# EPFL-IMOS/simple-SFOD

Measured on AMD Instinct MI355X. Metric: teacher+student train images/s on 1024x2048 synthetic, higher is better.
Workload: dtype bf16x3

## Files before the change

include/sfod_hip.h:

```cpp
#ifndef SFOD_HIP_H
#define SFOD_HIP_H
#include <stdint.h>
#ifdef __cplusplus
extern "C" {
#endif

#define SFOD_F32 0
#define SFOD_BF16 1
#define SFOD_BF16X3 2
#define SFOD_F16X3 3

int sfod_version(void);
const char* sfod_last_error(void);

int sfod_preprocess(const void* const* img_ptrs, const int32_t* sizes, int B, int Hp, int Wp,
                    int Cpad, const float* mean3, const float* std3, void* out, int dt,
                    void* stream);

int sfod_hflip_u8(const void* src, void* dst, int C, int H, int W, void* stream);

int sfod_resize_bilinear_u8(const void* src, void* dst, int C, int H, int W, int h, int w,
                            const int32_t* hbounds, const int32_t* hcoef, int ksize_h,
                            const int32_t* vbounds, const int32_t* vcoef, int ksize_v, int flip,
                            void* stream);
// ... 11 lines not shown
int sfod_conv_fwd_ws(const void* x, const void* w, const uint32_t* w_absmax, const float* bias, void* y, int B, int H,
                     int W, int Cin, int Cout, int ksize, int ldy, int act, float* stats, int dt, int out_dt,
                     void* stream);
int64_t sfod_conv_fwd_scratch_bytes(int B, int H, int W, int Cin, int Cout, int ksize, int dt, int out_dt, int with_stats);
int sfod_conv_fwd_scratch(const void* x, const void* w, const uint32_t* w_absmax, const float* bias, void* y, int B, int H,
                          int W, int Cin, int Cout, int ksize, int ldy, int act, float* stats, int dt, int out_dt,
                          void* scratch, int64_t scratch_bytes, void* stream);
int sfod_conv_stats_blocks(int B, int H, int W, int Cin, int Cout, int ksize, int dt);
int sfod_set_conv_algo(int algo);
int sfod_conv_dgrad_bnred_blocks(int B, int H, int W, int Cin, int Cout, int dt);
int sfod_conv_dgrad_bnred(const void* x, const void* w, void* dz, int B, int H, int W, int Cin, int Cout, int dt,
                          const float* y, const float* mean, const float* invstd, const float* gamma,
                          const float* beta, float* red_ws, void* stream);
int sfod_conv_fwd_bnin_supported(int B, int H, int W, int Cin, int Cout, int dt);
int sfod_conv_fwd_bnin(const float* x_pre, const float* in_mean, const float* in_invstd, const float* in_gamma,
                       const float* in_beta, const void* w, const float* bias, float* y, int B, int H, int W, int Cin,
                       int Cout, int ldy, int act, float* stats, int dt, void* stream);
int sfod_set_gemm_tile(int tile);
int sfod_set_conv3x3_variant(int variant);
int sfod_last_conv_kernel(char* buf, int n);
int sfod_set_deterministic(int on);
int sfod_get_deterministic(void);
int sfod_set_conv3x3_m16(int on);
int sfod_set_wgrad3x3_pipe(int on);
int sfod_conv_fwd_algo(int B, int H, int W, int Cin, int Cout, int ksize, int dt);

int sfod_conv_first_supported(int B, int H, int W, int Cin, int Cout, int dt, int ldy);
int sfod_conv_first_fused(const void* x, const void* w, const float* bias, const float* scale,
                          const float* shift, void* y, float* stats, int B, int H, int W, int ldy,
                          int act, int dt, void* stream);
int sfod_conv_first_fused_ws(const void* x, const void* w, const uint32_t* w_absmax, const float* bias,
                             const float* scale, const float* shift, void* y, float* stats, int B, int H, int W,
                             int ldy, int act, int dt, void* stream);

int64_t sfod_conv_wgrad_ws_bytes(int B, int H, int W, int Cin, int Cout, int ksize, int lddy, int dt);
int sfod_conv_wgrad(const void* x, const void* dy, float* dw, int B, int H, int W, int Cin,
                    int Cout, int ksize, int lddy, int dt, void* ws, int64_t ws_bytes, void* stream);
int sfod_conv_wgrad_oihw_supported(int B, int H, int W, int Cin, int Cout, int ksize, int lddy, int dt);
int sfod_conv_wgrad_oihw(const void* x, const void* dy, float* dw_oihw, int B, int H, int W, int Cin,
                         int Cout, int ksize, int lddy, int dt, int accumulate, void* ws,
                         int64_t ws_bytes, void* stream);
int sfod_conv_first_wgrad_bn_supported(int B, int H, int W, int Cin, int Cout, int pool, int dt, int y_dt);
int sfod_conv_first_wgrad_bn(const void* x, const void* dz, const void* y, const float* mean, const float* invstd,
                             const float* gamma, const float* beta, const float* dgamma, const float* dbeta,
                             float* dw, int B, int H, int W, int Cin, int Cout, int dt, int oihw, int accumulate,
                             void* ws, int64_t ws_bytes, void* stream);
int sfod_set_first_wgrad_fused(int on);

int sfod_pack_conv_weight(const float* w_oihw, void* w_packed, int Cout, int Cin, int ksize,
                          int CinPad, int rot180, int dt, void* stream);
int sfod_pack_conv_weight_ws(const float* w_oihw, void* w_packed, uint32_t* absmax, int Cout, int Cin, int ksize,
                             int CinPad, int rot180, int dt, void* stream);
int sfod_pack_conv_weights_blocks(int Cout, int Cin, int ksize, int innerPad, int rot180);
int sfod_pack_conv_weights_multi(const int64_t* desc, int n, int total_blocks, int dt, void* stream);
int sfod_pack_conv_weights_multi_ws(const int64_t* desc, int n, int total_blocks, int dt, uint32_t* absmax ,
                                    void* stream);
int sfod_unpack_conv_wgrad(const float* dw_packed, float* dw_oihw, int Cout, int Cin, int ksize,
                           int CinPad, int accumulate, void* stream);
int sfod_pack_fc_weight(const float* w, void* out, int N, int K, int chw_c, int transpose, int dt,
                        void* stream);
int sfod_unpack_fc_wgrad(const float* dw_packed, float* dw, int N, int K, int chw_c,
                         int accumulate, void* stream);
int sfod_pack_fc_weight_ld(const float* w, void* out, int N, int K, int chw_c, int transpose, int ld,
                           int dt, void* stream);
int sfod_pack_fc_weight_ld_ws(const float* w, void* out, uint32_t* absmax, int N, int K, int chw_c, int transpose,
                              int ld, int dt, void* stream);
// ... 251 lines not shown
```

simple-sfod_amd/csrc/conv_first.hip:

```cpp
#include "conv_internal.h"
#include <type_traits>

typedef __attribute__((ext_vector_type(8))) __bf16 bf16x8;
typedef __attribute__((ext_vector_type(16))) float f32x16;

namespace {

constexpr int TH = 8, TW = 32, PW = TW + 2, PH = TH + 2;
constexpr int PATCH_BYTES = PH * PW * 16;
constexpr int STG_OFF = 5632;
constexpr int STG_PITCH = 144;
constexpr int SRED_OFF = STG_OFF + 4 * 64 * STG_PITCH;
constexpr int LDS_BYTES = SRED_OFF + 4 * 64 * 2 * 4 + 16;
constexpr int X3_PATCH_BYTES = PH * PW * 32;
constexpr int X3_W_OFF = 11008;
constexpr int X3_W_BYTES = 5 * 2 * 2 * 64 * 16;
constexpr int X3_STG_OFF = X3_W_OFF + X3_W_BYTES;
constexpr int X3_FP = 272;
constexpr int X3_SRED_OFF = X3_STG_OFF + 4 * 16 * X3_FP;
constexpr int X3_LDS_BYTES = X3_SRED_OFF + 4 * 64 * 2 * 4 + 16;

struct F1Args {
  const bf16_t* x;
  const bf16_t* w;
  const float* bias;
  const float* scale;
  const float* shift;
  void* y;
  float* stats;
  int B, H, W, ldy, act;
  int tiles_y, tiles_x, ntiles;
  const unsigned* wamax;
};

__global__ void __launch_bounds__(256)
k_conv_first(F1Args a) {
  __shared__ __attribute__((aligned(16))) unsigned char smem[LDS_BYTES];
  const int lane = threadIdx.x & 63;
  const int wave = __builtin_amdgcn_readfirstlane(threadIdx.x >> 6);
  const int h = lane >> 5, l31 = lane & 31;

  bf16x8 bq[2][5];
#pragma unroll
  for (int j = 0; j < 2; ++j)
#pragma unroll
    for (int s = 0; s < 5; ++s) {
      const int tap = 2 * s + h;
      uint4 v = make_uint4(0, 0, 0, 0);
      if (tap < 9) v = *reinterpret_cast<const uint4*>(a.w + ((j * 32 + l31) * 9 + tap) * 8);
      bq[j][s] = __builtin_bit_cast(bf16x8, v);
    }
  float bcol[2], scol[2], hcol[2];
#pragma unroll
  for (int j = 0; j < 2; ++j) {
    bcol[j] = a.bias ? a.bias[j * 32 + l31] : 0.f;
    scol[j] = a.scale ? a.scale[j * 32 + l31] : 1.f;
    hcol[j] = a.shift ? a.shift[j * 32 + l31] : 0.f;
  }
  const float lo = (a.act == 1) ? 0.f : -__builtin_inff();

  for (int tile = blockIdx.x; tile < a.ntiles; tile += gridDim.x) {
    int t = tile;
    const int txi = t % a.tiles_x;
    t /= a.tiles_x;
    const int tyi = t % a.tiles_y;
// ... 115 lines not shown
        }
        q += __shfl_xor(q, 32);
        if (h == 0) {
          sred[(wave * 64 + j * 32 + l31) * 2 + 0] = sm;
          sred[(wave * 64 + j * 32 + l31) * 2 + 1] = q;
        }
      }
      if (lane == 0) scnt[wave] = (float)cnt;
      __syncthreads();
      if (threadIdx.x < 64) {
        const int col = threadIdx.x;
        double n_tot = 0.0, s_tot = 0.0;
#pragma unroll
        for (int k = 0; k < 4; ++k) { n_tot += (double)scnt[k]; s_tot += (double)sred[(k * 64 + col) * 2]; }
        const double mu = n_tot > 0.0 ? s_tot / n_tot : 0.0;
        double m2 = 0.0;
#pragma unroll
        for (int k = 0; k < 4; ++k) {
          const double nk = (double)scnt[k];
          if (nk > 0.0) {
            const double d = (double)sred[(k * 64 + col) * 2] / nk - mu;
            m2 += (double)sred[(k * 64 + col) * 2 + 1] + nk * d * d;
          }
        }
        a.stats[((int64_t)tile * 2 + 0) * 64 + col] = (float)s_tot;
        a.stats[((int64_t)tile * 2 + 1) * 64 + col] = (float)m2;
        if (col == 0) a.stats[(int64_t)a.ntiles * 2 * 64 + tile] = (float)n_tot;
      }
    }
  }
}

template <int FMT>
__global__ void __launch_bounds__(256) __attribute__((amdgpu_waves_per_eu(3, 3)))
k_conv_first_x3(F1Args a) {
  using pair_t = typename std::conditional<FMT == 2, splith_t, split_t>::type;
  const float winv = (FMT == 2 && a.wamax != nullptr) ? winv_from_absmax(*a.wamax) : 1.0f;
  __shared__ __attribute__((aligned(16))) unsigned char smem[X3_LDS_BYTES];
  const int lane = threadIdx.x & 63;
  const int wave = __builtin_amdgcn_readfirstlane(threadIdx.x >> 6);
  const int h = lane >> 5, l31 = lane & 31;
  for (int e = threadIdx.x; e < 5 * 2 * 64; e += 256) {
    const int ln = e & 63, j = (e >> 6) & 1, ks = e >> 7;
    const int tap = 2 * ks + (ln >> 5);
    uint4 vh = make_uint4(0, 0, 0, 0), vl = vh;
    if (tap < 9) {
      const uint4* p = reinterpret_cast<const uint4*>(a.w + ((j * 32 + (ln & 31)) * 9 + tap) * 16);
      vh = p[0];
      vl = p[1];
    }
    *reinterpret_cast<uint4*>(smem + X3_W_OFF + (((ks * 2 + j) * 2 + 0) * 64 + ln) * 16) = vh;
    *reinterpret_cast<uint4*>(smem + X3_W_OFF + (((ks * 2 + j) * 2 + 1) * 64 + ln) * 16) = vl;
  }
  float bcol[2], scol[2], hcol[2];
#pragma unroll
  for (int j = 0; j < 2; ++j) {
    bcol[j] = a.bias ? a.bias[j * 32 + l31] : 0.f;
    scol[j] = a.scale ? a.scale[j * 32 + l31] : 1.f;
    hcol[j] = a.shift ? a.shift[j * 32 + l31] : 0.f;
  }
  const float lo = (a.act == 1) ? 0.f : -__builtin_inff();
  const bool zsplit = (a.scale != nullptr);

  for (int tile = blockIdx.x; tile < a.ntiles; tile += gridDim.x) {
    int t = tile;
    const int txi = t % a.tiles_x;
    t /= a.tiles_x;
    const int tyi = t % a.tiles_y;
    const int b = t / a.tiles_y;
    const int x0 = txi * TW, y0 = tyi * TH;
    const bf16_t* ximg = a.x + (int64_t)b * a.H * a.W * 16;
// ... 128 lines not shown
            q += ((vmask[i] >> r) & 1u) ? d * d : 0.f;
          }
        q += __shfl_xor(q, 32);
        if (h == 0) {
          sred[(wave * 64 + j * 32 + l31) * 2 + 0] = sm;
          sred[(wave * 64 + j * 32 + l31) * 2 + 1] = q;
        }
      }
      if (lane == 0) scnt[wave] = (float)cnt;
      __syncthreads();
      if (threadIdx.x < 64) {
        const int col = threadIdx.x;
        double n_tot = 0.0, s_tot = 0.0;
#pragma unroll
        for (int k = 0; k < 4; ++k) { n_tot += (double)scnt[k]; s_tot += (double)sred[(k * 64 + col) * 2]; }
        const double mu = n_tot > 0.0 ? s_tot / n_tot : 0.0;
        double m2 = 0.0;
#pragma unroll
        for (int k = 0; k < 4; ++k) {
          const double nk = (double)scnt[k];
          if (nk > 0.0) {
            const double d = (double)sred[(k * 64 + col) * 2] / nk - mu;
            m2 += (double)sred[(k * 64 + col) * 2 + 1] + nk * d * d;
          }
        }
        a.stats[((int64_t)tile * 2 + 0) * 64 + col] = (float)s_tot;
        a.stats[((int64_t)tile * 2 + 1) * 64 + col] = (float)m2;
        if (col == 0) a.stats[(int64_t)a.ntiles * 2 * 64 + tile] = (float)n_tot;
      }
    }
  }
}

}

int sfod_f1_nblk(int B, int H, int W) { return B * ((H + TH - 1) / TH) * ((W + TW - 1) / TW); }

int sfod_f1_launch(const void* x, const void* w, const float* bias, void* y, float* stats, int B, int H, int W,
                   int ldy, int act, hipStream_t s, const float* scale, const float* shift, int split, const unsigned* wamax) {
  F1Args a;
  a.wamax = wamax;
  a.x = (const bf16_t*)x; a.w = (const bf16_t*)w; a.bias = bias; a.y = y; a.stats = stats;
  a.scale = scale; a.shift = shift;
  a.B = B; a.H = H; a.W = W; a.ldy = ldy; a.act = act;
  a.tiles_y = (H + TH - 1) / TH; a.tiles_x = (W + TW - 1) / TW;
  a.ntiles = B * a.tiles_y * a.tiles_x;
  const int resident = split ? 256 * 3 : 256 * 8;
  int grid = a.ntiles < resident ? a.ntiles : resident;
  sfod_note_conv_kernel(split == 2 ? "k_conv_first_x3<2>" : (split ? "k_conv_first_x3<1>" : "k_conv_first"));
  if (split == 2) hipLaunchKernelGGL(k_conv_first_x3<2>, dim3(grid), dim3(256), 0, s, a);
  else if (split) hipLaunchKernelGGL(k_conv_first_x3<1>, dim3(grid), dim3(256), 0, s, a);
  else hipLaunchKernelGGL(k_conv_first, dim3(grid), dim3(256), 0, s, a);
  return sfod_check_launch("conv_first");
}

SFOD_DEFINE_F16_POLL(sfod_f16_poll_first)
```

simple-sfod_amd/csrc/conv_internal.h:

```cpp
#pragma once
#include "common.h"

struct P3Plan {
  int ok;
  int G;
  int FM;
  int TH, TW;
  int tiles_y, tiles_x, tiles_n;
  int nblk;
  int m16;
};
P3Plan sfod_p3_plan(int B, int H, int W, int Cin, int Cout, int pairs = 0);
struct P3BnRed {
  const float* y;
  const float* mean;
  const float* invstd;
  const float* gamma;
  const float* beta;
  float* ws;
};
struct P3BnIn {
  const float* mean;
  const float* invstd;
  const float* gamma;
// ... 12 lines not shown
  int co_tiles, ci_tiles;
  int tiles_per_split, nsplit, nslab;
  int64_t ws_bytes;
  int w64;
};
W3Plan sfod_w3_plan(int B, int H, int W, int Cin, int Cout, int lddy, int split = 0);
int sfod_w3_launch(const W3Plan& p, const void* x, const void* dy, float* dw, void* ws, int B, int H, int W,
                   int Cin, int Cout, int lddy, int out_mode, hipStream_t s, int split = 0);

struct W3BnApply {
  const float* dz;
  const float* y;
  const float* mean;
  const float* invstd;
  const float* gamma;
  const float* beta;
  const float* dgamma;
  const float* dbeta;
};
bool sfod_w3_bn_ok(const W3Plan& p, int Cin, int Cout);
int sfod_w3_bn_launch(const W3Plan& p, const void* x, const W3BnApply& bn, float* dw, void* ws, int B, int H, int W,
                      int out_mode, hipStream_t s);

bool sfod_deterministic();

void sfod_f16_poll_elementwise(unsigned* out, hipStream_t s);
void sfod_f16_poll_roi(unsigned* out, hipStream_t s);
void sfod_f16_poll_first(unsigned* out, hipStream_t s);
void sfod_f16_poll_stem(unsigned* out, hipStream_t s);
void sfod_f16_poll_gn(unsigned* out, hipStream_t s);
void sfod_f16_poll_cda(unsigned* out, hipStream_t s);

int sfod_f1_nblk(int B, int H, int W);
int sfod_f1_launch(const void* x, const void* w, const float* bias, void* y, float* stats, int B, int H, int W,
                   int ldy, int act, hipStream_t s, const float* scale = nullptr, const float* shift = nullptr, int split = 0,
                   const unsigned* wamax = nullptr);
```

simple-sfod_amd/csrc/gemm_conv.hip:

```cpp
#include "conv_internal.h"
#include <algorithm>

typedef __attribute__((ext_vector_type(8))) __bf16 bf16x8;
typedef __attribute__((ext_vector_type(4))) short s16x4;
typedef __attribute__((ext_vector_type(8))) short s16x8;
typedef __attribute__((ext_vector_type(16))) float f32x16;
typedef __attribute__((ext_vector_type(4))) float f32x4;

#define LDS_PTR(p) ((__attribute__((address_space(3))) void*)(p))
#define GLB_PTR(p) ((const __attribute__((address_space(1))) void*)(p))

__device__ __attribute__((aligned(16))) unsigned int g_zero_page[64];

struct ConvArgs {
  int M;
  int H, W;
  int Cin;
  int Cout;
  int ks;
  int cpt_shift;
  int kchunks;
  int ldy;
  int act;
  const unsigned* wamax;
// ... 625 lines not shown
    }
  }
#undef TILE
  sfod_set_error("conv_fwd: tile shape %d is not built for these operands", (int)tile);
  return SFOD_EBADARG;
}

template <typename T, typename OutT, int SPLIT = 0>
static int launch_conv_fwd(const ConvFwdPlan& p, const void* x, const void* w, const float* bias, void* y, float* stats,
                           const ConvArgs& a, hipStream_t s) {
  if (p.ut) return launch_tile<T, OutT, true, SPLIT>(p.tile, x, w, bias, y, stats, a, s);
  return launch_tile<T, OutT, false, SPLIT>(p.tile, x, w, bias, y, stats, a, s);
}

extern "C" int sfod_conv_first_supported(int B, int H, int W, int Cin, int Cout, int dt, int ldy) {
  if (!(conv_shape_fits(B, H, W, Cin, Cout, 3) && sfod_ints_ok({ldy}))) return 0;
  return conv_fwd_plan(B, H, W, Cin, Cout, 3, dt, sfod_is_pairs(dt) ? SFOD_F32 : dt, ldy, true, 0).kind == CONV_FIRST ? 1 : 0;
}

extern "C" int sfod_conv_first_fused(const void* x, const void* w, const float* bias, const float* scale,
                                     const float* shift, void* y, float* stats, int B, int H, int W, int ldy,
                                     int act, int dt, void* stream) {
  SFOD_REQUIRE_EXTENTS("conv_first_fused", B, H, W, ldy);
  return sfod_conv_first_fused_ws(x, w, nullptr, bias, scale, shift, y, stats, B, H, W, ldy, act, dt, stream);
}

extern "C" int sfod_conv_first_fused_ws(const void* x, const void* w, const uint32_t* w_absmax, const float* bias,
                                        const float* scale, const float* shift, void* y, float* stats, int B, int H,
                                        int W, int ldy, int act, int dt, void* stream) {
  sfod_note_conv_kernel(nullptr);
  SFOD_REQUIRE(conv_shape_fits(B, H, W, 8, 64, 3) && sfod_ints_ok({ldy}), "conv_first_fused: negative or oversized extent");
  SFOD_REQUIRE(x != nullptr && w != nullptr, "conv_first_fused: null operand");
  SFOD_REQUIRE(w_absmax == nullptr || dt == SFOD_F16X3, "conv_first: scaled weights are an SFOD_F16X3 format");
  SFOD_REQUIRE(sfod_conv_first_supported(B, H, W, 8, 64, dt, ldy),
               "conv_first_fused: shape not served by the first-layer kernel (sfod_conv_first_supported)");
  SFOD_REQUIRE(y != nullptr || stats != nullptr, "conv_first_fused: nothing to produce");
  SFOD_REQUIRE((scale == nullptr) == (shift == nullptr), "conv_first_fused: scale and shift come together");
  return sfod_f1_launch(x, w, bias, y, stats, B, H, W, ldy, act, (hipStream_t)stream, scale, shift, split_code(dt), w_absmax);
}

extern "C" int sfod_conv_fwd_scratch(const void* x, const void* w, const uint32_t* w_absmax, const float* bias, void* y,
                                     int B, int H, int W, int Cin, int Cout, int ksize, int ldy, int act, float* stats,
                                     int dt, int out_dt, void* scratch, int64_t scratch_bytes, void* stream) {
  sfod_note_conv_kernel(nullptr);
  SFOD_REQUIRE(conv_shape_fits(B, H, W, Cin, Cout, ksize) && sfod_ints_ok({ldy}) && sfod_i64s_ok({scratch_bytes}),
               "conv_fwd: negative or oversized extent");
  SFOD_REQUIRE(x != nullptr && w != nullptr && y != nullptr, "conv_fwd: null operand (x, w, y)");
  SFOD_REQUIRE(act >= 0 && act <= 2, "conv_fwd: unknown act");
  SFOD_REQUIRE(out_dt == SFOD_F32 || out_dt == SFOD_BF16 || sfod_is_pairs(out_dt), "conv_fwd: unknown out_dt");
  SFOD_REQUIRE(w_absmax == nullptr || dt == SFOD_F16X3, "conv: scaled weights are an SFOD_F16X3 format");
  SFOD_REQUIRE(ksize == 1 || ksize == 3, "conv: ksize must be 1 or 3");
  SFOD_REQUIRE(ldy >= Cout, "conv: ldy < Cout");
  const int E = (dt == SFOD_F32) ? 4 : 8;
  SFOD_REQUIRE(dt == SFOD_F32 || dt == SFOD_BF16 || sfod_is_pairs(dt), "conv: unknown dt");
  SFOD_REQUIRE(Cin % E == 0, "conv: Cin must be a multiple of the 16-byte chunk (operand pairs: of 8)");
  SFOD_REQUIRE(!sfod_is_pairs(dt) || out_dt == SFOD_F32, "conv: operand pairs write fp32");
  if ((int64_t)B * H * W == 0) return 0;
  SFOD_REQUIRE(dt != SFOD_F32 || out_dt == SFOD_F32, "conv: fp32 compute writes fp32");
  const ConvFwdPlan p = conv_fwd_plan(B, H, W, Cin, Cout, ksize, dt, out_dt, ldy, stats != nullptr,
                                      scratch != nullptr ? scratch_bytes : 0);
  SFOD_REQUIRE(p.kind != CONV_NONE, "conv_fwd: negative or oversized extent");
  const bool as_query = ldy == Cout && out_dt == (sfod_is_pairs(dt) ? SFOD_F32 : dt);
  SFOD_REQUIRE(stats == nullptr || as_query || p.stats_blocks == sfod_conv_stats_blocks(B, H, W, Cin, Cout, ksize, dt),
               "conv_fwd: with this ldy / out_dt the launch writes another number of statistics blocks than "
               "sfod_conv_stats_blocks answers (it assumes dense rows and the operands' own output type)");
  hipStream_t s = (hipStream_t)stream;
  const int split = split_code(dt);
  Cin = phys_ch(dt, Cin);
  switch (p.kind) {
    case CONV_FIRST:
      return sfod_f1_launch(x, w, bias, y, stats, B, H, W, ldy, act, s, nullptr, nullptr, split, w_absmax);
// ... 726 lines not shown
```

simple-sfod_amd/modeling/backbone_vgg.py:

```python
import os

import torch
import torch.nn as nn

from .. import native
from .offchain import OffChain
from ..registry import BACKBONE_REGISTRY
from ..structures import ShapeSpec

VGG16 = [64, 64, "M", 128, 128, "M", 256, 256, 256, "M", 512, 512, 512, "M", 512, 512, 512, "M"]
STAGE_SLICES = [(0, 7), (7, 14), (14, 24), (24, 34), (34, 44)]


def make_layers(cfg_list, batch_norm=False):
    layers = []
    in_channels = 3
    for v in cfg_list:
        if v == "M":
            layers += [nn.MaxPool2d(kernel_size=2, stride=2)]
        else:
            conv2d = nn.Conv2d(in_channels, v, kernel_size=3, padding=1)
            if batch_norm:
                layers += [conv2d, nn.BatchNorm2d(v), nn.ReLU(inplace=True)]
            else:
# ... 180 lines not shown
            if pending is not None:
                yb, mb, ib, bnb = pending
                pending = None
                B, H, W, _ = yb.shape
                y, stats = native.conv_fwd_bnin(yb, mb, ib, bnb.weight.detach(), bnb.bias.detach(), wp, conv.bias.detach(),
                                                cout, want_stats=True)
                mean, invstd = finalize(stats, bn, cout, B * H * W)
                if self._defer_bn(li, y, fwd_w, save, training):
                    pending = (y, mean, invstd, bn)
                    continue
                x = native.bn_relu_pool_fwd(y, mean, invstd, bn.weight.detach(), bn.bias.detach(), pool, out_dtype=x.dtype)
                if stage_end:
                    outs.append(x)
                continue
            B, H, W, _ = x.shape
            if (li == 0 and training and not save and not pool and not stage_end and self.fuse_first
                    and native.conv_first_supported(x, cout)):
                stats = native.conv_first_stats(x, wp, conv.bias.detach())
                mean, invstd = finalize(stats, bn, cout, B * H * W)
                scale = bn.weight.detach() * invstd
                shift = bn.bias.detach() - mean * scale
                x = native.conv_first_apply(x, wp, conv.bias.detach(), scale, shift, relu=True)
                continue
            if training:
                y, stats = native.conv_fwd(x, wp, conv.bias.detach(), cout, 3, want_stats=True)
                mean, invstd = finalize(stats, bn, cout, B * H * W)
            else:
                y = native.conv_fwd(x, wp, conv.bias.detach(), cout, 3)
                mean = bn.running_mean
                invstd = torch.rsqrt(bn.running_var + self.bn_eps)
            if self._defer_bn(li, y, fwd_w, save, training):
                pending = (y, mean, invstd, bn)
                continue
            zz = native.bn_relu_pool_fwd(y, mean, invstd, bn.weight.detach(), bn.bias.detach(), pool,
                                         out_dtype=x.dtype, with_grad_operand=save)
            z, z_g = zz if save else (zz, None)
            if save:
                saved.append((x_g, y, mean, invstd))
            x, x_g = z, z_g
            if stage_end:
                outs.append(z)
        return saved, outs

    def _backward_impl(self, saved, out_grads):
        hook = getattr(self, "_pre_backward", None)
        if hook is not None:
            hook()
        dtype = self.grad_dtype
        pgrads = [None] * (4 * len(self._plan))
        stage_of = []
        s = 0
        for i, (_, _, _, stage_end) in enumerate(self._plan):
            stage_of.append(s if stage_end else None)
            if stage_end:
                s += 1
        dz = dz_red = None
        off = OffChain(self.wgrad_stream and dz_dev_is_cuda(out_grads))
        mid_hook = getattr(self, "_mid_backward", None)
        mid_layer = self._first_layer_of_stage(getattr(self, "_mid_stage", 2)) if mid_hook is not None else -1
        for li in range(len(self._plan) - 1, -1, -1):
            conv, bn, pool, stage_end = self._plan[li]
            x, y, mean, invstd = saved[li]
            if stage_end and out_grads[stage_of[li]] is not None:
                g = out_grads[stage_of[li]].permute(0, 2, 3, 1).to(native.out_dtype_of(dtype)).contiguous()
                dz = g if dz is None else native.add_(dz, g)
            if dz is None:
                continue
            gsink, bsink = native.grad_sink(bn.weight), native.grad_sink(bn.bias)
# ... 48 lines not shown
```

simple-sfod_amd/native.py:

```python
import collections
import ctypes
import math
import os
import re
import warnings

import torch

warnings.filterwarnings("ignore", message="ComplexHalf support is experimental")

_HERE = os.path.dirname(os.path.abspath(__file__))
HEADER = os.path.join(os.path.dirname(_HERE), "include", "sfod_hip.h")
SO_PATH = os.environ.get("SFOD_HIP_LIB", os.path.join(_HERE, "lib", "libsfod_hip.so"))

F32, BF16, BF16X3, F16X3 = 0, 1, 2, 3

SPLIT_DTYPE = torch.complex32
SPLITH_DTYPE = torch.uint32
PAIR_DTYPES = (SPLIT_DTYPE, SPLITH_DTYPE)

COMPUTE_MODES = {"fp32": F32, "bf16": BF16, "bf16x3": BF16X3, "f16x3": F16X3}


def mode_dt(name):
# ... 680 lines not shown
    B, H, W, cin = y_pre.shape
    return bool(query("sfod_conv_fwd_bnin_supported", B, H, W, cin, cout, BF16X3))


def conv_fwd_bnin(y_pre, mean, invstd, gamma, beta, w_packed, bias, cout, act=0, want_stats=False):
    B, H, W, cin = y_pre.shape
    y = torch.empty((B, H, W, cout), dtype=torch.float32, device=y_pre.device)
    stats = _stats_buffer(B, H, W, cin, cout, 3, BF16X3, y_pre.device) if want_stats else None
    call("sfod_conv_fwd_bnin", y_pre, mean, invstd, gamma, beta, w_packed, bias, y, B, H, W, cin, cout, cout, act, stats,
         BF16X3, timer_name="sfod_conv_fwd", flops=2.0 * B * H * W * cout * 9 * cin, tag=":patch3x3")
    return (y, stats) if want_stats else y


def conv_first_supported(x, cout):
    if x.dim() != 4 or x.dtype not in (torch.bfloat16,) + PAIR_DTYPES:
        return False
    B, H, W, cin = x.shape
    return bool(query("sfod_conv_first_supported", B, H, W, cin, cout, dt_of(x), cout))


def conv_first_stats(x, w_packed, bias):
    B, H, W, cin = x.shape
    stats = _stats_buffer(B, H, W, cin, 64, 3, dt_of(x), x.device)
    call("sfod_conv_first_fused_ws", x, w_packed, wscale_of(w_packed), bias, None, None, None, stats, B, H, W, 64, 0,
         dt_of(x))
    return stats


def conv_first_apply(x, w_packed, bias, scale, shift, relu=True):
    B, H, W, cin = x.shape
    z = torch.empty(B, H, W, 64, dtype=x.dtype, device=x.device)
    call("sfod_conv_first_fused_ws", x, w_packed, wscale_of(w_packed), bias, scale, shift, z, None, B, H, W, 64,
         1 if relu else 0, dt_of(x))
    return z


_ws_cache = {}


def _workspace(dev, nbytes):
    key = (dev, _stream())
    cur = _ws_cache.get(key)
    if cur is None or cur.numel() < nbytes:
        cur = torch.empty(int(nbytes), dtype=torch.uint8, device=dev)
        _ws_cache[key] = cur
    return cur


def _wgrad_call(name, args, extents, flops, timer_name=None):
    nbytes = query("sfod_conv_wgrad_ws_bytes", *extents)
    ws = _workspace(args[0].device, nbytes) if nbytes > 0 else None
    call(name, *args, ws, nbytes, timer_name=timer_name, flops=flops)


def conv_wgrad(x, dy, cout, ksize, dw_packed=None, operand=None):
    operand = operand or x.dtype
    x, dy = as_operand(x, operand), as_operand(dy, operand)
    dt = dt_of(x)
    if x.dim() == 2:
        B, H, W, cin = x.shape[0], 1, 1, x.shape[1]
    else:
        B, H, W, cin = x.shape
    lddy = dy.shape[-1]
    cout_k = (cout + 7) // 8 * 8 if dt in (BF16X3, F16X3) else cout
    assert cout_k <= lddy, "dy narrower than the padded output-channel count"
    if dw_packed is None or cout_k != cout:
# ... 808 lines not shown
```

Before: 162.4.

## Add software-pipelined persistent first-conv kernel and recompute fused BN-apply epilogue

Rewrites the split-precision first-layer conv as a persistent kernel that prefetches the next tile's input into registers while computing the current one. It double-buffers the patch and stats reduction areas in stats-only mode and defers the per-tile stats combine to the next iteration. It also adds a BN-apply mode that recomputes the first conv and applies BatchNorm+ReLU directly to produce z, replacing the separate bn_relu_pool_fwd pass over the f32 output. This trades extra MFMA work and more LDS per workgroup for fewer memory passes and better latency hiding.

```diff
diff --git a/include/sfod_hip.h b/include/sfod_hip.h
--- a/include/sfod_hip.h
+++ b/include/sfod_hip.h
@@ -67,6 +67,14 @@
 int sfod_conv_first_fused_ws(const void* x, const void* w, const uint32_t* w_absmax, const float* bias,
                              const float* scale, const float* shift, void* y, float* stats, int B, int H, int W,
                              int ldy, int act, int dt, void* stream);
+int sfod_conv_first_stats_blocks(int B, int H, int W);
+int sfod_set_conv_first_pipe(int on);
+int sfod_set_conv_first_grid(int n);
+int sfod_conv_first_bn_apply_supported(int B, int H, int W, int Cin, int Cout, int pool_flags, int dt, int y_dt);
+int sfod_conv_first_bn_apply(const void* x, const void* w, const float* bias, const float* mean, const float* invstd,
+                             const float* gamma, const float* beta, void* z, int B, int H, int W, int ldz, int dt,
+                             void* stream);
+int sfod_set_first_apply_recompute(int on);
 
 int64_t sfod_conv_wgrad_ws_bytes(int B, int H, int W, int Cin, int Cout, int ksize, int lddy, int dt);
 int sfod_conv_wgrad(const void* x, const void* dy, float* dw, int B, int H, int W, int Cin,
diff --git a/simple-sfod_amd/csrc/conv_first.hip b/simple-sfod_amd/csrc/conv_first.hip
--- a/simple-sfod_amd/csrc/conv_first.hip
+++ b/simple-sfod_amd/csrc/conv_first.hip
@@ -18,7 +18,13 @@
 constexpr int X3_STG_OFF = X3_W_OFF + X3_W_BYTES;
 constexpr int X3_FP = 272;
 constexpr int X3_SRED_OFF = X3_STG_OFF + 4 * 16 * X3_FP;
-constexpr int X3_LDS_BYTES = X3_SRED_OFF + 4 * 64 * 2 * 4 + 16;
+constexpr int X3_SRED_BYTES = 4 * 64 * 2 * 4 + 16;
+constexpr int X3_LDS_BYTES = X3_SRED_OFF + X3_SRED_BYTES;
+constexpr int X3_PIPE_LDS_BYTES = X3_SRED_OFF + 2 * X3_SRED_BYTES;
+static_assert(X3_PATCH_BYTES <= 4 * 16 * X3_FP, "the second patch buffer lives in the staging area");
+static_assert(3 * X3_PIPE_LDS_BYTES <= 160 * 1024, "3 workgroups per CU");
+
+enum { F1_PLAIN = 0, F1_STATS = 1, F1_Y = 2, F1_AFFINE = 3, F1_BN = 4 };
 
 struct F1Args {
   const bf16_t* x;
@@ -31,6 +37,10 @@
   int B, H, W, ldy, act;
   int tiles_y, tiles_x, ntiles;
   const unsigned* wamax;
+  const float* mean;
+  const float* invstd;
+  const float* gamma;
+  const float* beta;
 };
 
 __global__ void __launch_bounds__(256)
@@ -212,11 +222,9 @@
 }
 
 template <int FMT>
-__global__ void __launch_bounds__(256) __attribute__((amdgpu_waves_per_eu(3, 3)))
-k_conv_first_x3(F1Args a) {
+__device__ __forceinline__ void f1_x3_plain(const F1Args& a, unsigned char* smem) {
   using pair_t = typename std::conditional<FMT == 2, splith_t, split_t>::type;
   const float winv = (FMT == 2 && a.wamax != nullptr) ? winv_from_absmax(*a.wamax) : 1.0f;
-  __shared__ __attribute__((aligned(16))) unsigned char smem[X3_LDS_BYTES];
   const int lane = threadIdx.x & 63;
   const int wave = __builtin_amdgcn_readfirstlane(threadIdx.x >> 6);
   const int h = lane >> 5, l31 = lane & 31;
@@ -411,25 +419,352 @@
   }
 }
 
+#pragma clang fp contract(off)
+
+__device__ __forceinline__ void f1_combine(const F1Args& a, const float* sred, int tile, int col, bool full) {
+  const float* scnt = sred + 4 * 64 * 2;
+  double n_tot = 0.0, s_tot = 0.0, m2 = 0.0;
+#pragma unroll
+  for (int k = 0; k < 4; ++k) s_tot += (double)sred[(k * 64 + col) * 2];
+  if (full) {
+    n_tot = 256.0;
+    const double mu = s_tot * (1.0 / 256.0);
+#pragma unroll
+    for (int k = 0; k < 4; ++k) {
+      const double d = (double)sred[(k * 64 + col) * 2] * (1.0 / 64.0) - mu;
+      m2 += __builtin_fma(d, 64.0 * d, (double)sred[(k * 64 + col) * 2 + 1]);
+    }
+  } else {
+#pragma unroll
+    for (int k = 0; k < 4; ++k) n_tot += (double)scnt[k];
+    const double mu = n_tot > 0.0 ? s_tot / n_tot : 0.0;
+#pragma unroll
+    for (int k = 0; k < 4; ++k) {
+      const double nk = (double)scnt[k];
+      if (nk > 0.0) {
+        const double d = (double)sred[(k * 64 + col) * 2] / nk - mu;
+        m2 += __builtin_fma(d, nk * d, (double)sred[(k * 64 + col) * 2 + 1]);
+      }
+    }
+  }
+  a.stats[((int64_t)tile * 2 + 0) * 64 + col] = (float)s_tot;
+  a.stats[((int64_t)tile * 2 + 1) * 64 + col] = (float)m2;
+  if (col == 0) a.stats[(int64_t)a.ntiles * 2 * 64 + tile] = (float)n_tot;
 }
 
+template <int FMT, int MODE>
+__device__ __forceinline__ void f1_x3_pipe(const F1Args& a, unsigned char* smem) {
+  using pair_t = typename std::conditional<FMT == 2, splith_t, split_t>::type;
+  constexpr bool DB = (MODE == F1_STATS);
+  const bool with_stats = MODE != F1_BN && a.stats != nullptr;
+  const float winv = (FMT == 2 && a.wamax != nullptr) ? winv_from_absmax(*a.wamax) : 1.0f;
+  const int tid = threadIdx.x, lane = tid & 63;
+  const int wave = __builtin_amdgcn_readfirstlane(tid >> 6);
+  const int h = lane >> 5, l31 = lane & 31;
+  const int G = gridDim.x;
+  int tile = blockIdx.x;
+  if (tile >= a.ntiles) return;
+  for (int e = tid; e < 5 * 2 * 64; e += 256) {
+    const int ln = e & 63, j = (e >> 6) & 1, ks = e >> 7;
+    const int tap = 2 * ks + (ln >> 5);
+    uint4 vh = make_uint4(0, 0, 0, 0), vl = vh;
+    if (tap < 9) {
+      const uint4* p = reinterpret_cast<const uint4*>(a.w + ((j * 32 + (ln & 31)) * 9 + tap) * 16);
+      vh = p[0];
+      vl = p[1];
+    }
+    *reinterpret_cast<uint4*>(smem + X3_W_OFF + (((ks * 2 + j) * 2 + 0) * 64 + ln) * 16) = vh;
+    *reinterpret_cast<uint4*>(smem + X3_W_OFF + (((ks * 2 + j) * 2 + 1) * 64 + ln) * 16) = vl;
+  }
+  float bcol[2], c0[2], c1[2], c2[2];
+#pragma unroll
+  for (int j = 0; j < 2; ++j) {
+    const int c = j * 32 + l31;
+    bcol[j] = a.bias ? a.bias[c] : 0.f;
+    c0[j] = c1[j] = c2[j] = 0.f;
+    if constexpr (MODE == F1_AFFINE) { c0[j] = a.scale[c]; c1[j] = a.shift[c]; }
+    if constexpr (MODE == F1_BN) { c0[j] = a.mean[c]; c1[j] = a.invstd[c] * a.gamma[c]; c2[j] = a.beta[c]; }
+  }
+  const float lo = (a.act == 1) ? 0.f : -__builtin_inff();
+
+  int cpyx[3], crel[3];
+#pragma unroll
+  for (int k = 0; k < 3; ++k) {
+    const int p = tid + 256 * k, pp = p >> 1, half = p & 1;
+    const int py = pp / PW, px = pp - py * PW;
+    cpyx[k] = (py << 8) | px;
+    crel[k] = (py * a.W + px) * 32 + half * 16;
+  }
+  const bool third = tid < PH * PW * 2 - 512;
+  int aoff[5];
+#pragma unroll
+  for (int s = 0; s < 5; ++s) {
+    const int tap = 2 * s + h;
+    const int ky = tap / 3, kx = tap - ky * 3;
+    aoff[s] = ((2 * wave + ky) * PW + l31 + kx) * 32;
+  }
+  const int tyx = a.tiles_y * a.tiles_x;
+  const int sb = G / tyx, sy = (G - sb * tyx) / a.tiles_x, sx = G - sb * tyx - sy * a.tiles_x;
+  int b = tile / tyx, tyi = (tile - b * tyx) / a.tiles_x, txi = tile - b * tyx - tyi * a.tiles_x;
+
+  uint4 pre[3];
+  auto fetch = [&](int fb, int fty, int ftx) {
+    const int ym = fty * TH - 1, xm = ftx * TW - 1;
+    const int64_t base = (((int64_t)fb * a.H + ym) * a.W + xm) * 32;
+#pragma unroll
+    for (int k = 0; k < 3; ++k) {
+      const int iy = ym + (cpyx[k] >> 8), ix = xm + (cpyx[k] & 255);
+      const bool ok = (k < 2 || third) && iy >= 0 && iy < a.H && ix >= 0 && ix < a.W;
+      const uint4 v = *reinterpret_cast<const uint4*>(reinterpret_cast<const unsigned char*>(a.x) + (ok ? base + crel[k] : 0));
+      pre[k] = ok ? v : make_uint4(0, 0, 0, 0);
+    }
+  };
+  fetch(b, tyi, txi);
+
+  float* const sred0 = reinterpret_cast<float*>(smem + X3_SRED_OFF);
+  int prev_tile = -1, it = 0;
+  bool prev_full = false;
+  for (;; ++it) {
+    const int x0 = txi * TW, y0 = tyi * TH;
+    unsigned char* patch = smem + ((DB && (it & 1)) ? X3_STG_OFF : 0);
+#pragma unroll
+    for (int k = 0; k < 3; ++k)
+      if (k < 2 || third) *reinterpret_cast<uint4*>(patch + (tid + 256 * k) * 16) = pre[k];
+    const int ntile = tile + G;
+    const bool more = ntile < a.ntiles;
+    int nb = b + sb, nty = tyi + sy, ntx = txi + sx;
+    if (ntx >= a.tiles_x) { ntx -= a.tiles_x; ++nty; }
+    if (nty >= a.tiles_y) { nty -= a.tiles_y; ++nb; }
+    if (more) fetch(nb, nty, ntx);
+    __syncthreads();
+    if (with_stats && prev_tile >= 0 && wave == ((it - 1) & 3))
+      f1_combine(a, sred0 + ((it - 1) & 1) * (X3_SRED_BYTES / 4), prev_tile, lane, prev_full);
+
+    f32x16 acc[2][2];
+#pragma unroll
+    for (int i = 0; i < 2; ++i)
+#pragma unroll
+      for (int j = 0; j < 2; ++j)
+#pragma unroll
+        for (int r = 0; r < 16; ++r) acc[i][j][r] = 0.f;
+#pragma unroll
+    for (int s = 0; s < 5; ++s) {
+      bf16x8 ah[2], al[2], bh[2], bl[2];
+#pragma unroll
+      for (int i = 0; i < 2; ++i) {
+        uint4 vh = make_uint4(0, 0, 0, 0), vl = vh;
+        if (s < 4 || h == 0) {
+          vh = *reinterpret_cast<const uint4*>(patch + aoff[s] + i * (PW * 32));
+          vl = *reinterpret_cast<const uint4*>(patch + aoff[s] + i * (PW * 32) + 16);
+        }
+        ah[i] = __builtin_bit_cast(bf16x8, vh);
+        al[i] = __builtin_bit_cast(bf16x8, vl);
+      }
+#pragma unroll
+      for (int j = 0; j < 2; ++j) {
+        bh[j] = __builtin_bit_cast(
+            bf16x8, *reinterpret_cast<const uint4*>(smem + X3_W_OFF + (((s * 2 + j) * 2 + 0) * 64 + lane) * 16));
+        bl[j] = __builtin_bit_cast(
+            bf16x8, *reinterpret_cast<const uint4*>(smem + X3_W_OFF + (((s * 2 + j) * 2 + 1) * 64 + lane) * 16));
+      }
+#pragma unroll
+      for (int i = 0; i < 2; ++i)
+#pragma unroll
+        for (int j = 0; j < 2; ++j) acc[i][j] = mfma_pairs<FMT>(ah[i], bl[j], acc[i][j]);
+#pragma unroll
+      for (int i = 0; i < 2; ++i)
+#pragma unroll
+        for (int j = 0; j < 2; ++j) acc[i][j] = mfma_pairs<FMT>(al[i], bh[j], acc[i][j]);
+#pragma unroll
+      for (int i = 0; i < 2; ++i)
+#pragma unroll
+        for (int j = 0; j < 2; ++j) acc[i][j] = mfma_pairs<FMT>(ah[i], bh[j], acc[i][j]);
+    }
+#pragma unroll
+    for (int i = 0; i < 2; ++i)
+#pragma unroll
+      for (int j = 0; j < 2; ++j)
+#pragma unroll
+        for (int r = 0; r < 16; ++r)
+          acc[i][j][r] = (FMT == 2) ? __builtin_fmaf(acc[i][j][r], winv, bcol[j]) : acc[i][j][r] + bcol[j];
+
+    const bool full = (y0 + TH <= a.H) && (x0 + TW <= a.W);
+    auto epilogue = [&](auto full_c) {
+      constexpr bool FULL = decltype(full_c)::value;
+      unsigned vmask[2] = {0xffffu, 0xffffu};
+      if constexpr (!FULL) {
+#pragma unroll
+        for (int i = 0; i < 2; ++i) {
+          unsigned m = 0;
+          const int iy = y0 + 2 * wave + i;
+#pragma unroll
+          for (int r = 0; r < 16; ++r) {
+            const int px = (r & 3) + 8 * (r >> 2) + 4 * h;
+            if (iy < a.H && x0 + px < a.W) m |= (1u << r);
+          }
+          vmask[i] = m;
+        }
+      }
+      if constexpr (MODE != F1_STATS) {
+        unsigned char* stg = smem + X3_STG_OFF + wave * (16 * X3_FP);
+#pragma unroll
+        for (int i = 0; i < 2; ++i) {
+          const int iy = y0 + 2 * wave + i;
+#pragma unroll
+          for (int qh = 0; qh < 2; ++qh) {
+#pragma unroll
+            for (int j = 0; j < 2; ++j)
+#pragma unroll
+              for (int rr = 0; rr < 8; ++rr) {
+                const int r = qh * 8 + rr;
+                const int ml = (rr & 3) + 8 * (rr >> 2) + 4 * h;
+                float o;
+                if constexpr (MODE == F1_AFFINE) {
+                  o = fmaxf(__builtin_fmaf(acc[i][j][r], c0[j], c1[j]), lo);
+                } else if constexpr (MODE == F1_BN) {
+                  const float yv = fmaxf(__builtin_fmaf(acc[i][j][r], 1.f, 0.f), -__builtin_inff());
+                  o = fmaxf(__builtin_fmaf(yv - c0[j], c1[j], c2[j]), 0.f);
+                } else {
+                  o = fmaxf(__builtin_fmaf(acc[i][j][r], 1.f, 0.f), lo);
+                }
+                *reinterpret_cast<float*>(stg + ml * X3_FP + (j * 32 + l31) * 4) = o;
+              }
+            if constexpr (MODE == F1_AFFINE || MODE == F1_BN) {
+#pragma unroll
+              for (int it2 = 0; it2 < 2; ++it2) {
+                const int row = it2 * 8 + (lane >> 3), gch = lane & 7;
+                const int ix = x0 + qh * 16 + row;
+                if (FULL || (iy < a.H && ix < a.W)) {
+                  const float4 v0 = *reinterpret_cast<const float4*>(stg + row * X3_FP + gch * 32);
+                  const float4 v1 = *reinterpret_cast<const float4*>(stg + row * X3_FP + gch * 32 + 16);
+                  const float f[8] = {v0.x, v0.y, v0.z, v0.w, v1.x, v1.y, v1.z, v1.w};
+                  split_store8(reinterpret_cast<pair_t*>(a.y) + (((int64_t)b * a.H + iy) * a.W + ix) * a.ldy + gch * 8, f);
+                }
+              }
+            } else {
+#pragma unroll
+              for (int it2 = 0; it2 < 4; ++it2) {
+                const int row = it2 * 4 + (lane >> 4), ch = lane & 15;
+                const int ix = x0 + qh * 16 + row;
+                if (FULL || (iy < a.H && ix < a.W))
+                  *reinterpret_cast<float4*>(reinterpret_cast<float*>(a.y) + (((int64_t)b * a.H + iy) * a.W + ix) * a.ldy + ch * 4) =
+                      *reinterpret_cast<const float4*>(stg + row * X3_FP + ch * 16);
+              }
+            }
+          }
+        }
+      }
+      if (with_stats) {
+        float* sred = sred0 + (it & 1) * (X3_SRED_BYTES / 4);
+        float* scnt = sred + 4 * 64 * 2;
+        int cnt = 64;
+        if constexpr (!FULL) {
+          cnt = __builtin_popcount(vmask[0]) + __builtin_popcount(vmask[1]);
+          cnt += __shfl_xor(cnt, 32);
+        }
+        const float inv = 1.f / (float)(cnt > 0 ? cnt : 1);
+#pragma unroll
+        for (int j = 0; j < 2; ++j) {
+          float sm = 0.f, q = 0.f;
+#pragma unroll
+          for (int i = 0; i < 2; ++i)
+#pragma unroll
+            for (int r = 0; r < 16; ++r) sm = sm + ((FULL || ((vmask[i] >> r) & 1u)) ? acc[i][j][r] : 0.f);
+          sm = sm + __shfl_xor(sm, 32);
+#pragma unroll
+          for (int i = 0; i < 2; ++i)
+#pragma unroll
+            for (int r = 0; r < 16; ++r) {
+              const float d = __builtin_fmaf(-inv, sm, acc[i][j][r]);
+              const float dd = d * d;
+              q = q + ((FULL || ((vmask[i] >> r) & 1u)) ? dd : 0.f);
+            }
+          q = q + __shfl_xor(q, 32);
+          if (h == 0) {
+            sred[(wave * 64 + j * 32 + l31) * 2 + 0] = sm;
+            sred[(wave * 64 + j * 32 + l31) * 2 + 1] = q;
+          }
+        }
+        if (lane == 0) scnt[wave] = (float)cnt;
+      }
+    };
+    if (full) epilogue(std::true_type{});
+    else epilogue(std::false_type{});
+
+    if (!DB) __syncthreads();
+    prev_full = full;
+    if (!more) break;
+    prev_tile = tile;
+    tile = ntile;
+    b = nb; tyi = nty; txi = ntx;
+  }
+  if (with_stats) {
+    if (DB) __syncthreads();
+    if (wave == (it & 3)) f1_combine(a, sred0 + (it & 1) * (X3_SRED_BYTES / 4), tile, lane, prev_full);
+  }
+}
+
+template <int FMT, int MODE>
+__global__ void __launch_bounds__(256) __attribute__((amdgpu_waves_per_eu(3, 3)))
+k_conv_first_x3(F1Args a) {
+  __shared__ __attribute__((aligned(16))) unsigned char smem[MODE == F1_PLAIN ? X3_LDS_BYTES : X3_PIPE_LDS_BYTES];
+  if constexpr (MODE == F1_PLAIN) f1_x3_plain<FMT>(a, smem);
+  else f1_x3_pipe<FMT, MODE>(a, smem);
+}
+
+}
+
+constexpr int F1_PIPE_MAX_W = 1 << 22;
+bool sfod_f1_bn_ok(int W) { return W <= F1_PIPE_MAX_W; }
+
 int sfod_f1_nblk(int B, int H, int W) { return B * ((H + TH - 1) / TH) * ((W + TW - 1) / TW); }
 
+static SfodKnob g_f1_pipe{"SFOD_F1_PIPE", 1, sfod_knob_bool};
+static SfodKnob g_f1_grid{"SFOD_F1_GRID", 0, [](int n) { return n > 0 ? n : 0; }};
+extern "C" int sfod_set_conv_first_pipe(int on) { g_f1_pipe.set(on); return 0; }
+extern "C" int sfod_set_conv_first_grid(int n) { g_f1_grid.set(n); return 0; }
+
+template <int FMT>
+static void f1_x3_dispatch(int mode, int grid, hipStream_t s, const F1Args& a) {
+  switch (mode) {
+    case F1_STATS: hipLaunchKernelGGL((k_conv_first_x3<FMT, F1_STATS>), dim3(grid), dim3(256), 0, s, a); break;
+    case F1_Y: hipLaunchKernelGGL((k_conv_first_x3<FMT, F1_Y>), dim3(grid), dim3(256), 0, s, a); break;
+    case F1_AFFINE: hipLaunchKernelGGL((k_conv_first_x3<FMT, F1_AFFINE>), dim3(grid), dim3(256), 0, s, a); break;
+    case F1_BN:
+      if constexpr (FMT == 1) hipLaunchKernelGGL((k_conv_first_x3<FMT, F1_BN>), dim3(grid), dim3(256), 0, s, a);
+      break;
+    default: hipLaunchKernelGGL((k_conv_first_x3<FMT, F1_PLAIN>), dim3(grid), dim3(256), 0, s, a); break;
+  }
+}
+
 int sfod_f1_launch(const void* x, const void* w, const float* bias, void* y, float* stats, int B, int H, int W,
-                   int ldy, int act, hipStream_t s, const float* scale, const float* shift, int split, const unsigned* wamax) {
+                   int ldy, int act, hipStream_t s, const float* scale, const float* shift, int split, const unsigned* wamax,
+                   const F1BnApply* bn) {
   F1Args a;
   a.wamax = wamax;
   a.x = (const bf16_t*)x; a.w = (const bf16_t*)w; a.bias = bias; a.y = y; a.stats = stats;
   a.scale = scale; a.shift = shift;
+  a.mean = bn ? bn->mean : nullptr; a.invstd = bn ? bn->invstd : nullptr;
+  a.gamma = bn ? bn->gamma : nullptr; a.beta = bn ? bn->beta : nullptr;
   a.B = B; a.H = H; a.W = W; a.ldy = ldy; a.act = act;
   a.tiles_y = (H + TH - 1) / TH; a.tiles_x = (W + TW - 1) / TW;
   a.ntiles = B * a.tiles_y * a.tiles_x;
-  const int resident = split ? 256 * 3 : 256 * 8;
+  if (a.ntiles == 0) return 0;  const int resident = split ? 256 * 3 : 256 * 8;
   int grid = a.ntiles < resident ? a.ntiles : resident;
+  const int cap = g_f1_grid.get();
+  if (cap > 0 && grid > cap) grid = cap;
   sfod_note_conv_kernel(split == 2 ? "k_conv_first_x3<2>" : (split ? "k_conv_first_x3<1>" : "k_conv_first"));
-  if (split == 2) hipLaunchKernelGGL(k_conv_first_x3<2>, dim3(grid), dim3(256), 0, s, a);
-  else if (split) hipLaunchKernelGGL(k_conv_first_x3<1>, dim3(grid), dim3(256), 0, s, a);
-  else hipLaunchKernelGGL(k_conv_first, dim3(grid), dim3(256), 0, s, a);
+  if (split) {
+    const bool pipe_ok = W <= F1_PIPE_MAX_W;
+    SFOD_REQUIRE(bn == nullptr || (y != nullptr && scale == nullptr && split == 1 && pipe_ok),
+                 "conv_first: BatchNorm epilogue on bf16 pairs");
+    const int mode = bn ? F1_BN : (!(g_f1_pipe.get() && pipe_ok) ? F1_PLAIN : (y == nullptr ? F1_STATS : (scale ? F1_AFFINE : F1_Y)));
+    if (split == 2) f1_x3_dispatch<2>(mode, grid, s, a);
+    else f1_x3_dispatch<1>(mode, grid, s, a);
+  } else {
+    SFOD_REQUIRE(bn == nullptr, "conv_first: BatchNorm epilogue on bf16 pairs");
+    hipLaunchKernelGGL(k_conv_first, dim3(grid), dim3(256), 0, s, a);
+  }
   return sfod_check_launch("conv_first");
 }
 
diff --git a/simple-sfod_amd/csrc/conv_internal.h b/simple-sfod_amd/csrc/conv_internal.h
--- a/simple-sfod_amd/csrc/conv_internal.h
+++ b/simple-sfod_amd/csrc/conv_internal.h
@@ -68,6 +68,13 @@
 void sfod_f16_poll_cda(unsigned* out, hipStream_t s);
 
 int sfod_f1_nblk(int B, int H, int W);
+bool sfod_f1_bn_ok(int W);
+struct F1BnApply {
+  const float* mean;
+  const float* invstd;
+  const float* gamma;
+  const float* beta;
+};
 int sfod_f1_launch(const void* x, const void* w, const float* bias, void* y, float* stats, int B, int H, int W,
                    int ldy, int act, hipStream_t s, const float* scale = nullptr, const float* shift = nullptr, int split = 0,
-                   const unsigned* wamax = nullptr);
+                   const unsigned* wamax = nullptr, const F1BnApply* bn = nullptr);
diff --git a/simple-sfod_amd/csrc/gemm_conv.hip b/simple-sfod_amd/csrc/gemm_conv.hip
--- a/simple-sfod_amd/csrc/gemm_conv.hip
+++ b/simple-sfod_amd/csrc/gemm_conv.hip
@@ -681,11 +681,38 @@
   SFOD_REQUIRE(conv_shape_fits(B, H, W, 8, 64, 3) && sfod_ints_ok({ldy}), "conv_first_fused: negative or oversized extent");
   SFOD_REQUIRE(x != nullptr && w != nullptr, "conv_first_fused: null operand");
   SFOD_REQUIRE(w_absmax == nullptr || dt == SFOD_F16X3, "conv_first: scaled weights are an SFOD_F16X3 format");
-  SFOD_REQUIRE(sfod_conv_first_supported(B, H, W, 8, 64, dt, ldy),
-               "conv_first_fused: shape not served by the first-layer kernel (sfod_conv_first_supported)");
+  SFOD_REQUIRE((dt == SFOD_BF16 || sfod_is_pairs(dt)) && ldy % 8 == 0,
+               "conv_first_fused: operands not served by the first-layer kernel (sfod_conv_first_supported)");
   SFOD_REQUIRE(y != nullptr || stats != nullptr, "conv_first_fused: nothing to produce");
   SFOD_REQUIRE((scale == nullptr) == (shift == nullptr), "conv_first_fused: scale and shift come together");
   return sfod_f1_launch(x, w, bias, y, stats, B, H, W, ldy, act, (hipStream_t)stream, scale, shift, split_code(dt), w_absmax);
+}
+
+extern "C" int sfod_conv_first_stats_blocks(int B, int H, int W) {
+  return conv_shape_fits(B, H, W, 8, 64, 3) ? sfod_f1_nblk(B, H, W) : 0;
+}
+
+static SfodKnob g_first_apply_recompute{"SFOD_FIRST_APPLY_RECOMPUTE", 1, sfod_knob_bool};
+extern "C" int sfod_set_first_apply_recompute(int on) { g_first_apply_recompute.set(on); return 0; }
+
+extern "C" int sfod_conv_first_bn_apply_supported(int B, int H, int W, int Cin, int Cout, int pool_flags, int dt, int y_dt) {
+  if (!g_first_apply_recompute.get() || !conv_shape_fits(B, H, W, Cin, Cout, 3)) return 0;
+  if (Cin != 8 || Cout != 64 || pool_flags != 0 || dt != SFOD_BF16X3 || y_dt != SFOD_F32 || !sfod_f1_bn_ok(W)) return 0;
+  return conv_query_plan(B, H, W, Cin, Cout, 3, dt).kind == CONV_FIRST ? 1 : 0;
+}
+
+extern "C" int sfod_conv_first_bn_apply(const void* x, const void* w, const float* bias, const float* mean,
+                                        const float* invstd, const float* gamma, const float* beta, void* z, int B, int H,
+                                        int W, int ldz, int dt, void* stream) {
+  sfod_note_conv_kernel(nullptr);
+  SFOD_REQUIRE(conv_shape_fits(B, H, W, 8, 64, 3) && sfod_ints_ok({ldz}), "conv_first_bn_apply: negative or oversized extent");
+  SFOD_REQUIRE(x != nullptr && w != nullptr && z != nullptr, "conv_first_bn_apply: null operand");
+  SFOD_REQUIRE(mean != nullptr && invstd != nullptr && gamma != nullptr && beta != nullptr,
+               "conv_first_bn_apply: null BatchNorm operand");
+  SFOD_REQUIRE(dt == SFOD_BF16X3 && ldz % 8 == 0 && ldz >= 64 && sfod_f1_bn_ok(W),
+               "conv_first_bn_apply: not served (sfod_conv_first_bn_apply_supported)");
+  const F1BnApply bn{mean, invstd, gamma, beta};
+  return sfod_f1_launch(x, w, bias, z, nullptr, B, H, W, ldz, 1, (hipStream_t)stream, nullptr, nullptr, 1, nullptr, &bn);
 }
 
 extern "C" int sfod_conv_fwd_scratch(const void* x, const void* w, const uint32_t* w_absmax, const float* bias, void* y,
diff --git a/simple-sfod_amd/modeling/backbone_vgg.py b/simple-sfod_amd/modeling/backbone_vgg.py
--- a/simple-sfod_amd/modeling/backbone_vgg.py
+++ b/simple-sfod_amd/modeling/backbone_vgg.py
@@ -236,8 +236,13 @@
             if self._defer_bn(li, y, fwd_w, save, training):
                 pending = (y, mean, invstd, bn)
                 continue
-            zz = native.bn_relu_pool_fwd(y, mean, invstd, bn.weight.detach(), bn.bias.detach(), pool,
-                                         out_dtype=x.dtype, with_grad_operand=save)
+            if li == 0 and save and native.conv_first_bn_apply_supported(x, y, cout, pool):
+                z = native.conv_first_bn_apply(x, wp, conv.bias.detach(), mean, invstd, bn.weight.detach(),
+                                               bn.bias.detach())
+                zz = (z, z)
+            else:
+                zz = native.bn_relu_pool_fwd(y, mean, invstd, bn.weight.detach(), bn.bias.detach(), pool,
+                                             out_dtype=x.dtype, with_grad_operand=save)
             z, z_g = zz if save else (zz, None)
             if save:
                 saved.append((x_g, y, mean, invstd))
diff --git a/simple-sfod_amd/native.py b/simple-sfod_amd/native.py
--- a/simple-sfod_amd/native.py
+++ b/simple-sfod_amd/native.py
@@ -736,6 +736,35 @@
     z = torch.empty(B, H, W, 64, dtype=x.dtype, device=x.device)
     call("sfod_conv_first_fused_ws", x, w_packed, wscale_of(w_packed), bias, scale, shift, z, None, B, H, W, 64,
          1 if relu else 0, dt_of(x))
+    return z
+
+
+def set_conv_first_pipe(on):
+    load().sfod_set_conv_first_pipe(int(on))
+
+
+def set_conv_first_grid(n):
+    load().sfod_set_conv_first_grid(int(n))
+
+
+def set_first_apply_recompute(on):
+    load().sfod_set_first_apply_recompute(int(on))
+
+
+def conv_first_bn_apply_supported(x, y, cout, pool, relu=True):
+    if x.dim() != 4 or y.dim() != 4 or not x.is_cuda or tuple(y.shape) != (*x.shape[:3], cout):
+        return False
+    if x.dtype not in PAIR_DTYPES:
+        return False
+    B, H, W, cin = x.shape
+    return bool(query("sfod_conv_first_bn_apply_supported", B, H, W, cin, cout, int(pool) | (0 if relu else 2), dt_of(x),
+                      dt_of(y)))
+
+
+def conv_first_bn_apply(x, w_packed, bias, mean, invstd, gamma, beta):
+    B, H, W, cin = x.shape
+    z = torch.empty(B, H, W, 64, dtype=x.dtype, device=x.device)
+    call("sfod_conv_first_bn_apply", x, w_packed, bias, mean, invstd, gamma, beta, z, B, H, W, 64, dt_of(x))
     return z
 
 
```

New measurement: 164.2 (median of 6 runs). +1.1%, better.
